# bxh1/VIDO-SLAM

Hardware: AMD Instinct MI355X
Metric: frames/sec end-to-end (flow+depth+track+local-BA) at 640x480; BA iters/sec (higher is better)
Workload: dtype f32

## Files before the change

vido-slam_amd/csrc/detpost.hip:

```cpp
#include "common.hpp"
#include <cfloat>

namespace {
typedef unsigned long long u64;

__device__ void block_sort_desc(u64* keys, int n)
{
    for (int k = 2; k <= n; k <<= 1)
        for (int j = k >> 1; j > 0; j >>= 1) {
            for (int t = threadIdx.x; t < n; t += blockDim.x) {
                const int x = t ^ j;
                if (x > t) {
                    const u64 a = keys[t], b = keys[x];
                    const bool up = (t & k) != 0;
                    if (up ? a > b : a < b) { keys[t] = b; keys[x] = a; }
                }
            }
            __syncthreads();
        }
}

__device__ int block_excl_scan(int v, int* wsum , int* total)
{
    const int lane = threadIdx.x & 63, wave = threadIdx.x >> 6, nw = blockDim.x >> 6;
// ... 182 lines not shown
        const u64 key = mkeys[t];
        int rank = q;
        for (int m = 0; m < Lv; m++) {
            if (m == l) continue;
            const u64* lst = mkeys + (size_t)m * K; int lo = 0, hi = s_cnt[m];
            while (lo < hi) { const int mid = (lo + hi) >> 1; if (lst[mid] > key) lo = mid + 1; else hi = mid; }
            rank += lo;
        }
        if (rank < n_final) {
            const int flat = (int)(0xffffffffu - (unsigned)key);
            for (int c = 0; c < 4; c++) out_boxes[4 * rank + c] = boxes[4 * (size_t)flat + c];
            out_scores[rank] = __uint_as_float((unsigned)(key >> 32));
        }
    }
    if (tid == 0) *n_valid = min(total, n_final);
}

__global__ __launch_bounds__(1024) void k_det_class_sort(const float* __restrict__ prob, const float* __restrict__ deltas, const float* __restrict__ proposals, const float* __restrict__ objectness,
                                                         int N, int nc, float thresh, float wx, float wy, float ww, float wh, float img_w, float img_h,
                                                         float* __restrict__ seg_boxes , int* __restrict__ order , int* __restrict__ seg_n)
{
    __shared__ u64 keys[1024];
    __shared__ int s_n;
    const int j = blockIdx.x + 1, tid = threadIdx.x;
    if (tid == 0) s_n = 0;
    __syncthreads();
    u64 key = 0;
    if (tid < N) {
        float s = prob[(size_t)tid * nc + j];
        if (objectness && objectness[tid] < 0.f) s = 0.f;
        if (s > thresh) { key = ((u64)__float_as_uint(s) << 32) | (u64)(0xffffffffu - (unsigned)tid); atomicAdd(&s_n, 1); }
    }
    keys[tid] = key;
    __syncthreads();
    block_sort_desc(keys, 1024);
    const int n = s_n;
    if (tid < N) {
        float* ob = seg_boxes + ((size_t)(j - 1) * N + tid) * 4; int* oo = order + (size_t)(j - 1) * N + tid;
        if (tid < n) {
            const int i = (int)(0xffffffffu - (unsigned)keys[tid]);
            const float* d = deltas + ((size_t)i * nc + j) * 4;
            decode_clip(proposals + 4 * (size_t)i, d[0], d[1], d[2], d[3], wx, wy, ww, wh, img_w, img_h, ob);
            *oo = i;
        } else { ob[0] = ob[1] = ob[2] = ob[3] = 0.f; *oo = 0; }
    }
    if (tid == 0) seg_n[j - 1] = n;
}

#define DT_STAGE 8192
__global__ __launch_bounds__(1024) void k_det_thresh(const float* __restrict__ prob, const int* __restrict__ order, const int* __restrict__ keep, const int* __restrict__ cnt,
                                                     int N, int nc, int kth, unsigned* __restrict__ thr_out)
{
    __shared__ unsigned hist[256];
    __shared__ unsigned stage[DT_STAGE];
    __shared__ int coff[1025];
    __shared__ unsigned s_prefix, s_kk;
    const int tid = threadIdx.x, lane = tid & 63, wave = tid >> 6, ncls = nc - 1;
    if (tid == 0) { int run = 0; for (int j = 0; j < ncls && j < 1024; j++) { coff[j] = run; run += cnt[j]; } coff[min(ncls, 1024)] = run; }
    __syncthreads();
    const unsigned total = (unsigned)coff[min(ncls, 1024)];
    if (kth <= 0 || total <= (unsigned)kth || ncls > 1024) { if (tid == 0) { thr_out[0] = 0u; thr_out[1] = total; } return; }
    const bool staged = total <= DT_STAGE;
    auto score_bits = [&](int j, int q) { const int i = order[(size_t)j * N + keep[(size_t)j * N + q]]; return __float_as_uint(prob[(size_t)i * nc + j + 1]); };
    if (staged) {
        for (int j = wave; j < ncls; j += 16) { const int c = coff[j + 1] - coff[j]; for (int q = lane; q < c; q += 64) stage[coff[j] + q] = score_bits(j, q); }
        __syncthreads();
    }
    unsigned prefix = 0, mask = 0;
    if (tid == 0) s_kk = (unsigned)kth;
    for (int shift = 24; shift >= 0; shift -= 8) {
        if (tid < 256) hist[tid] = 0;
        __syncthreads();
        if (staged) { for (unsigned t = tid; t < total; t += 1024) { const unsigned u = stage[t]; if ((u & mask) == prefix) atomicAdd(&hist[(u >> shift) & 255u], 1u); } }
        else for (int j = wave; j < ncls; j += 16) { const int c = coff[j + 1] - coff[j]; for (int q = lane; q < c; q += 64) { const unsigned u = score_bits(j, q); if ((u & mask) == prefix) atomicAdd(&hist[(u >> shift) & 255u], 1u); } }
        __syncthreads();
        if (tid == 0) { unsigned kk = s_kk, d; pick_digit_desc(hist, kk, d); s_kk = kk; s_prefix = prefix | (d << shift); }
        __syncthreads();
        prefix = s_prefix; mask |= 0xffu << shift;
    }
    if (tid == 0) { thr_out[0] = prefix; thr_out[1] = total; }
}

__global__ __launch_bounds__(1024) void k_det_emit(const float* __restrict__ prob, const float* __restrict__ seg_boxes, const int* __restrict__ order, const int* __restrict__ keep,
                                                   const int* __restrict__ cnt, int N, int nc, const unsigned* __restrict__ thr, int emit, int* __restrict__ class_counts, int cap,
                                                   float* __restrict__ out_boxes, float* __restrict__ out_scores, long long* __restrict__ out_labels, int* __restrict__ n_det)
{
    __shared__ int flag[1024]; __shared__ int spos[1024]; __shared__ int wsum[17];
    const int j = blockIdx.x, tid = threadIdx.x, ncls = nc - 1;
    const unsigned T = thr[0];
    flag[tid] = 0; spos[tid] = 0;
    __syncthreads();
    const int c = cnt[j];
    for (int q = tid; q < c; q += 1024) {
        const int p = keep[(size_t)j * N + q], i = order[(size_t)j * N + p];
        if (__float_as_uint(prob[(size_t)i * nc + j + 1]) >= T) { flag[i] = 1; spos[i] = p; }
    }
    __syncthreads();
    int total = 0;
    const int rank = block_excl_scan(tid < N ? flag[tid] : 0, wsum, &total);
    if (!emit) { if (tid == 0) class_counts[j] = total; return; }
    int off = 0, all = 0;
    for (int jj = 0; jj < ncls; jj++) { const int t = class_counts[jj]; if (jj < j) off += t; all += t; }
    if (tid < N && flag[tid]) {
        const int slot = off + rank;
        if (slot < cap) {
            const float* b = seg_boxes + ((size_t)j * N + spos[tid]) * 4;
            for (int k = 0; k < 4; k++) out_boxes[4 * slot + k] = b[k];
            out_scores[slot] = prob[(size_t)tid * nc + j + 1]; out_labels[slot] = (long long)(j + 1);
        }
    }
    if (j == 0) {
        for (int s = min(all, cap) + tid; s < cap; s += 1024) { for (int k = 0; k < 4; k++) out_boxes[4 * s + k] = 0.f; out_scores[s] = 0.f; out_labels[s] = 0; }
        if (tid == 0) *n_det = all;
    }
}
}

extern "C" {

int vido_rpn_select(vido_ctx* ctx, int n_levels, const float* const* logits, const float* const* deltas, const int* h, const int* w, const int* stride, const float* cell_anchors,
                    int A, int K, int img_w, int img_h, float* boxes_out, float* scores_out, int32_t* n_out)
{
    if (!ctx) return VIDO_E_INVALID;
    if (n_levels < 1 || n_levels > 8 || A < 1 || A > 4 || K < 1 || K > 1024 || !logits || !deltas || !h || !w || !stride || !cell_anchors || !boxes_out || !scores_out || !n_out)
        return vido_set_error(ctx, VIDO_E_INVALID, "rpn_select: bad arguments (<= 8 levels, <= 4 anchors per cell, K <= 1024)");
    HIP_TRY(ctx, hipSetDevice(ctx->device));
    hipStream_t st = ctx->has_ext_stream ? ctx->ext_stream : ctx->stream;
    RpnLevels L; memset(&L, 0, sizeof L); int maxn = 0; int n_of[8] = {0, 0, 0, 0, 0, 0, 0, 0};
    for (int l = 0; l < n_levels; l++) {
// ... 80 lines not shown
```

vido-slam_amd/csrc/nets.hip:

```cpp
#include "common.hpp"
#include <numeric>

#define CORR_CH 8
__global__ __launch_bounds__(256) void k_correlation(const float* __restrict__ f1, const float* __restrict__ f2, int C, int H, int W, int s,
                                                     int Ho, int Wo, float* __restrict__ out, int nsplit, int cper)
{
    __shared__ float t2[CORR_CH][22][23];
    const int tx = threadIdx.x & 15, ty = threadIdx.x >> 4, b = blockIdx.z / nsplit, split = blockIdx.z - b * nsplit;
    const int c_lo = split * cper, c_hi = min(C, c_lo + cper);
    const int x = blockIdx.x * 16 + tx, y = blockIdx.y * 16 + ty;
    const bool valid = x < Wo && y < Ho;
    float acc[49];
#pragma unroll
    for (int k = 0; k < 49; k++) acc[k] = 0.f;
    const size_t plane = (size_t)H * W;
    for (int c0 = c_lo; c0 < c_hi; c0 += CORR_CH) {
        const int nc = min(CORR_CH, c_hi - c0);
        for (int i = threadIdx.x; i < nc * 22 * 22; i += 256) {
            const int cc = i / (22 * 22), r = (i / 22) % 22, q = i % 22;
            const int yy = (blockIdx.y * 16 + r - 3), xx = (blockIdx.x * 16 + q - 3);
            float v = 0.f;
            if (yy >= 0 && yy < Ho && xx >= 0 && xx < Wo) v = f2[((size_t)b * C + c0 + cc) * plane + (size_t)(yy * s) * W + xx * s];
            t2[cc][r][q] = v;
        }
// ... 178 lines not shown
        const int ph = bin / PW, pw = bin - ph * PW;
        float acc = 0.f;
        if (SR == 2) {
            int o[4][4]; float w[4][4], v[4][4]; bool out[4];
#pragma unroll
            for (int s2 = 0; s2 < 4; s2++) {
                const int iy = s2 >> 1, ix = s2 & 1;
                const float y = sh + ph * bh + (float)(iy + .5f) * bh / (float)gh, x = sw + pw * bw + (float)(ix + .5f) * bw / (float)gw;
                out[s2] = taps(y, x, o[s2][0], o[s2][1], o[s2][2], o[s2][3], w[s2][0], w[s2][1], w[s2][2], w[s2][3]);
            }
#pragma unroll
            for (int s2 = 0; s2 < 4; s2++)
#pragma unroll
                for (int t = 0; t < 4; t++) v[s2][t] = d[(size_t)o[s2][t] * C];
#pragma unroll
            for (int s2 = 0; s2 < 4; s2++) acc += out[s2] ? 0.f : (w[s2][0] * v[s2][0] + w[s2][1] * v[s2][1] + w[s2][2] * v[s2][2] + w[s2][3] * v[s2][3]);
        } else {
            for (int iy = 0; iy < gh; iy++) {
                const float y = sh + ph * bh + (float)(iy + .5f) * bh / (float)gh;
                for (int ix = 0; ix < gw; ix++) {
                    const float x = sw + pw * bw + (float)(ix + .5f) * bw / (float)gw;
                    int o1, o2, o3, o4; float w1, w2, w3, w4;
                    if (taps(y, x, o1, o2, o3, o4, w1, w2, w3, w4)) { acc += 0.f; continue; }
                    const float v1 = d[(size_t)o1 * C], v2 = d[(size_t)o2 * C], v3 = d[(size_t)o3 * C], v4 = d[(size_t)o4 * C];
                    acc += (w1 * v1 + w2 * v2 + w3 * v3 + w4 * v4);
                }
            }
        }
        rl_tile[lane * pitch + bin] = acc / count;
    }
    __syncthreads();
    const int nc = min(64, C - c0), total = nc * nbin;
    float* o = out + ((size_t)i * C + c0) * nbin;
    for (int e = threadIdx.x; e < total; e += 256) { const int cc = e / nbin; o[e] = rl_tile[cc * pitch + (e - cc * nbin)]; }
}
__global__ __launch_bounds__(256) void k_nchw_to_nhwc(const float* __restrict__ src, int C, int HW, float* __restrict__ dst)
{
    __shared__ float t[64][65];
    const int p0 = blockIdx.x * 64, c0 = blockIdx.y * 64, b = blockIdx.z, lane = threadIdx.x & 63, q = threadIdx.x >> 6;
    const float* s = src + (size_t)b * C * HW; float* d = dst + (size_t)b * HW * C;
    for (int k = q; k < 64; k += 4) if (c0 + k < C && p0 + lane < HW) t[k][lane] = s[(size_t)(c0 + k) * HW + p0 + lane];
    __syncthreads();
    for (int k = q; k < 64; k += 4) if (p0 + k < HW && c0 + lane < C) d[(size_t)(p0 + k) * C + c0 + lane] = t[lane][k];
}

__device__ __forceinline__ void tile_of(int t, int nb, int& rb, int& cb)
{
    int r = (int)((2.0f * nb + 1.0f - sqrtf((2.0f * nb + 1.0f) * (2.0f * nb + 1.0f) - 8.0f * (float)t)) * 0.5f);
    r = max(0, min(r, nb - 1));
    while (r > 0 && r * nb - r * (r - 1) / 2 > t) r--;
    while ((r + 1) * nb - (r + 1) * r / 2 <= t) r++;
    rb = r; cb = r + (t - (r * nb - r * (r - 1) / 2));
}
__device__ __forceinline__ void nms_tile(const float* __restrict__ boxes, const int* __restrict__ group, int n, float thresh, unsigned long long* __restrict__ mask, int col_blocks, int rb, int cb, int lane)
{
    const int col = cb * 64 + lane; const bool cv = col < n;
    const float4 b = cv ? *(const float4*)(boxes + 4 * (size_t)col) : make_float4(0.f, 0.f, 0.f, 0.f);
    const float Sb = (b.z - b.x + 1) * (b.w - b.y + 1);
    const int gb = (group && cv) ? group[col] : 0;
    const int rows = min(n - rb * 64, 64);
    unsigned long long mine = 0;
    for (int i = 0; i < rows; i++) {
        const float* a = boxes + 4 * (size_t)(rb * 64 + i);
        const float a0 = a[0], a1 = a[1], a2 = a[2], a3 = a[3];
        const int ga = group ? group[rb * 64 + i] : 0;
        const float left = fmaxf(a0, b.x), right = fminf(a2, b.z), top = fmaxf(a1, b.y), bottom = fminf(a3, b.w);
        const float w = fmaxf(right - left + 1, 0.f), h = fmaxf(bottom - top + 1, 0.f), inter = w * h;
        const float Sa = (a2 - a0 + 1) * (a3 - a1 + 1);
        const bool hit = cv && ga == gb && inter / (Sa + Sb - inter) > thresh;
        unsigned long long word = __ballot(hit);
        if (rb == cb) word &= i >= 63 ? 0ull : ~((2ull << i) - 1ull);
        if (lane == i) mine = word;
    }
    if (lane < rows) mask[(size_t)(rb * 64 + lane) * col_blocks + cb] = mine;
}
__global__ __launch_bounds__(256) void k_nms_mask(const float* __restrict__ boxes, const int* __restrict__ group , int n, float thresh,
                                                 unsigned long long* __restrict__ mask, int col_blocks)
{
    const int t = __builtin_amdgcn_readfirstlane(blockIdx.x * 4 + (threadIdx.x >> 6)), nb = col_blocks;
    if (t >= nb * (nb + 1) / 2) return;
    int rb, cb; tile_of(t, nb, rb, cb);
    nms_tile(boxes, group, n, thresh, mask, col_blocks, rb, cb, threadIdx.x & 63);
}
__global__ __launch_bounds__(64) void k_nms_sweep(const unsigned long long* __restrict__ mask, int n, int col_blocks, int* __restrict__ keep, int* __restrict__ n_keep)
{
    const int lane = threadIdx.x;
    int cnt = 0;
    unsigned long long remv[16];
    const int wpl = (col_blocks + 63) / 64;
    for (int k = 0; k < 16; k++) remv[k] = 0;
    for (int i = 0; i < n; i++) {
        const int nblock = i >> 6, inblock = i & 63;
        const int owner = nblock & 63, slot = nblock >> 6;
        unsigned long long word = 0;
#pragma unroll
        for (int k = 0; k < 16; k++) if (k == slot) word = remv[k];
        word = __shfl(word, owner, 64);
        if (!(word & (1ULL << inblock))) {
            if (lane == 0) keep[cnt] = i;
            cnt++;
            const unsigned long long* p = mask + (size_t)i * col_blocks;
#pragma unroll
            for (int k = 0; k < 16; k++) if (k < wpl) { const int w = k * 64 + lane; if (w >= nblock && w < col_blocks) remv[k] |= p[w]; }
        }
    }
    if (lane == 0) *n_keep = cnt;
}

__global__ __launch_bounds__(64) void k_nms_sweep_seg(const unsigned long long* __restrict__ mask, const int* __restrict__ seg_off, const int* __restrict__ seg_n, int col_blocks,
                                                      int* __restrict__ keep, int* __restrict__ n_keep, int keep_stride)
{
    const int g = blockIdx.x, lane = threadIdx.x;
    const int n = seg_n[g];
    const unsigned long long* M = mask + (size_t)seg_off[g] * col_blocks;
    int* kp = keep + (size_t)g * keep_stride;
    const int cb = (n + 63) >> 6;
    unsigned long long remv[16];
#pragma unroll
    for (int k = 0; k < 16; k++) remv[k] = 0;
    int cnt = 0;
    for (int blk = 0; blk < cb; blk++) {
        const int owner = blk & 63, slot = blk >> 6, rows = min(n - blk * 64, 64);
        unsigned long long word = 0;
#pragma unroll
        for (int k = 0; k < 16; k++) if (k == slot) word = remv[k];
        word = __shfl(word, owner, 64);
        const unsigned long long diag = lane < rows ? M[(size_t)(blk * 64 + lane) * col_blocks + blk] : 0ull;
        const uint32_t dlo = (uint32_t)diag, dhi = (uint32_t)(diag >> 32);
        unsigned long long alive = ~word;
        if (rows < 64) alive &= (1ull << rows) - 1ull;
        unsigned long long keepmask = 0;
        while (alive) {
            const int j = __builtin_ctzll(alive);
            keepmask |= 1ull << j;
            const unsigned long long dj = (unsigned long long)(uint32_t)__builtin_amdgcn_readlane((int)dlo, j) | ((unsigned long long)(uint32_t)__builtin_amdgcn_readlane((int)dhi, j) << 32);
            alive &= ~dj; alive &= ~(1ull << j);
        }
        if ((keepmask >> lane) & 1ull) kp[cnt + __popcll(keepmask & ((1ull << lane) - 1ull))] = blk * 64 + lane;
        cnt += __popcll(keepmask);
        const bool mine = (keepmask >> lane) & 1ull;
        const unsigned long long* prow = M + (size_t)(blk * 64 + lane) * col_blocks;
        for (int w0 = blk + 1; w0 < cb; w0 += 4) {
            unsigned long long v[4];
#pragma unroll
            for (int u = 0; u < 4; u++) v[u] = (mine && w0 + u < cb) ? prow[w0 + u] : 0ull;
#pragma unroll
            for (int u = 0; u < 4; u++) {
                uint32_t lo = (uint32_t)v[u], hi = (uint32_t)(v[u] >> 32);
#pragma unroll
                for (int o = 32; o >= 1; o >>= 1) { lo |= (uint32_t)__shfl_xor((int)lo, o, 64); hi |= (uint32_t)__shfl_xor((int)hi, o, 64); }
                const int w = w0 + u;
                if (w < cb && lane == (w & 63)) {
                    const unsigned long long r = (unsigned long long)lo | ((unsigned long long)hi << 32);
#pragma unroll
                    for (int k = 0; k < 16; k++) if (k == (w >> 6)) remv[k] |= r;
                }
            }
        }
    }
    for (int i = cnt + lane; i < keep_stride; i += 64) kp[i] = -1;
    if (lane == 0) n_keep[g] = cnt;
}
__global__ __launch_bounds__(256) void k_nms_mask_seg(const float* __restrict__ boxes, const int* __restrict__ group, const int* __restrict__ seg_off, const int* __restrict__ seg_n,
                                                     float thresh, unsigned long long* __restrict__ mask, int col_blocks)
{
    const int g = blockIdx.y, n = seg_n[g], off = seg_off[g];
    const int nb = (n + 63) >> 6, t = __builtin_amdgcn_readfirstlane(blockIdx.x * 4 + (threadIdx.x >> 6));
    if (t >= nb * (nb + 1) / 2) return;
    int rb, cb; tile_of(t, nb, rb, cb);
    nms_tile(boxes + 4 * (size_t)off, group ? group + off : nullptr, n, thresh, mask + (size_t)off * col_blocks, col_blocks, rb, cb, threadIdx.x & 63);
}

struct PasteDet { int x0, y0, w, h, label; float rw, rh; };
__global__ __launch_bounds__(256) void k_paste_prepare(const float* __restrict__ boxes, const int64_t* __restrict__ labels, int n, int M, int padding, PasteDet* __restrict__ det)
{
    const int i = blockIdx.x * blockDim.x + threadIdx.x;
    if (i >= n) return;
    const float scale = (float)((double)(M + 2 * padding) / (double)M);
    const float* b = boxes + 4 * (size_t)i;
    const float wh = (b[2] - b[0]) * 0.5f * scale, hh = (b[3] - b[1]) * 0.5f * scale;
    const float xc = (b[2] + b[0]) * 0.5f, yc = (b[3] + b[1]) * 0.5f;
    const int x0 = (int)(xc - wh), y0 = (int)(yc - hh), x1 = (int)(xc + wh), y1 = (int)(yc + hh);
    PasteDet d; d.x0 = x0; d.y0 = y0; d.w = max(x1 - x0 + 1, 1); d.h = max(y1 - y0 + 1, 1); d.label = (int)labels[i];
    const int Mp = M + 2 * padding;
    d.rw = (float)Mp / (float)d.w; d.rh = (float)Mp / (float)d.h;
    det[i] = d;
}
__global__ __launch_bounds__(256) void k_paste_label(const float* __restrict__ masks , const PasteDet* __restrict__ det, int n, int M, int padding, float thresh,
                                                     int H, int W, uint8_t* __restrict__ out)
{
    __shared__ PasteDet sd[128];
    const int x = blockIdx.x * 32 + (threadIdx.x & 31), y = blockIdx.y * 8 + (threadIdx.x >> 5);
    const int Mp = M + 2 * padding;
    unsigned acc = 0;
    for (int d0 = 0; d0 < n; d0 += 128) {
        __syncthreads();
        if ((int)threadIdx.x < min(128, n - d0)) sd[threadIdx.x] = det[d0 + threadIdx.x];
        __syncthreads();
        if (x < W && y < H) {
            for (int k = 0; k < min(128, n - d0); k++) {
                const PasteDet d = sd[k];
                const int u = x - d.x0, v = y - d.y0;
                if (u < 0 || v < 0 || u >= d.w || v >= d.h) continue;
                float sy = d.rh * ((float)v + 0.5f) - 0.5f; if (sy < 0.f) sy = 0.f;
                float sx = d.rw * ((float)u + 0.5f) - 0.5f; if (sx < 0.f) sx = 0.f;
                const int iy = (int)sy, ix = (int)sx; const int iyp = iy < Mp - 1 ? 1 : 0, ixp = ix < Mp - 1 ? 1 : 0;
                const float ly = sy - (float)iy, lx = sx - (float)ix, hy = 1.f - ly, hx = 1.f - lx;
                const float* m = masks + (size_t)(d0 + k) * M * M;
                auto at = [&](int yy, int xx) -> float { yy -= padding; xx -= padding; return (yy < 0 || xx < 0 || yy >= M || xx >= M) ? 0.f : m[yy * M + xx]; };
                const float val = hy * (hx * at(iy, ix) + lx * at(iy, ix + ixp)) + ly * (hx * at(iy + iyp, ix) + lx * at(iy + iyp, ix + ixp));
                if (val > thresh) acc += (unsigned)d.label;
            }
        }
    }
    if (x < W && y < H) out[(size_t)y * W + x] = (uint8_t)acc;
}

__global__ void k_zero_i32(int32_t* __restrict__ p, int n)
{
    const int i = blockIdx.x * blockDim.x + threadIdx.x;
    if (i < n) p[i] = 0;
}
__global__ __launch_bounds__(256) void k_paste_instance(const float* __restrict__ masks , const PasteDet* __restrict__ det, int n, int M, int padding, float thresh,
// ... 173 lines not shown
    if (w >= W || h >= H) return;
    const size_t hw = (size_t)H * W, o = (size_t)h * W + w;
    const float* dp = dist + (size_t)b * ND * hw + o;
    float e[ND]; float m = -INFINITY;
#pragma unroll
    for (int c = 0; c < ND; c++) { const float v = dp[(size_t)c * hw]; e[c] = -(v * v); m = fmaxf(m, e[c]); }
    const float* fxp = flow + (size_t)b * 2 * hw; const float* fyp = fxp + hw;
    float s = 0.f, ax = 0.f, ay = 0.f;
#pragma unroll
    for (int c = 0; c < ND; c++) {
        const float p = expf(e[c] - m);
        s += p;
        const int yy = h + c / K - PAD, xx = w + c % K - PAD;
        const bool in = yy >= 0 && yy < H && xx >= 0 && xx < W;
        const size_t q = in ? (size_t)yy * W + xx : 0;
        const float ux = in ? fxp[q] : 0.f, uy = in ? fyp[q] : 0.f;
        ax += wx[c] * (p * ux); ay += wy[c] * (p * uy);
    }
    const float div = 1.0f / s;
    out[(size_t)b * 2 * hw + o] = (ax + bx[0]) * div;
    out[(size_t)b * 2 * hw + hw + o] = (ay + by[0]) * div;
}

__global__ __launch_bounds__(256) void k_deconv4s2_dw(const float* __restrict__ in, const float* __restrict__ wgt , int C, int H, int W, float slope, float* __restrict__ out)
{
    const int OW = 2 * W, OH = 2 * H;
    const int ox = blockIdx.x * 64 + (threadIdx.x & 63), oy = blockIdx.y * 4 + (threadIdx.x >> 6), bc = blockIdx.z, c = bc % C;
    if (ox >= OW || oy >= OH) return;
    const float* ip = in + (size_t)bc * H * W; const float* wp = wgt + 16 * c;
    const int ky0 = (oy + 1) & 1, kx0 = (ox + 1) & 1, iy0 = (oy + 1 - ky0) >> 1, ix0 = (ox + 1 - kx0) >> 1;
    float acc = 0.f;
#pragma unroll
    for (int a = 0; a < 2; a++) {
        const int iy = iy0 - a, ky = ky0 + 2 * a;
#pragma unroll
        for (int b = 0; b < 2; b++) {
            const int ix = ix0 - b, kx = kx0 + 2 * b;
            if (iy >= 0 && iy < H && ix >= 0 && ix < W) { float v = ip[(size_t)iy * W + ix]; v = v > 0.f ? v : v * slope; acc += v * wp[ky * 4 + kx]; }
        }
    }
    out[((size_t)bc * OH + oy) * OW + ox] = acc;
}

static int roi_lds_limit(vido_ctx* ctx, size_t lds)
{
    static size_t have = 48 * 1024;
    if (lds <= have) return VIDO_OK;
    HIP_TRY(ctx, hipFuncSetAttribute((const void*)k_roi_align_nhwc<2>, hipFuncAttributeMaxDynamicSharedMemorySize, (int)lds));
    HIP_TRY(ctx, hipFuncSetAttribute((const void*)k_roi_align_nhwc<0>, hipFuncAttributeMaxDynamicSharedMemorySize, (int)lds));
    have = lds;
    return VIDO_OK;
}

extern "C" {

int vido_correlation(vido_ctx* ctx, const float* first, const float* second, int B, int C, int H, int W, int stride, float* out, int on_device)
{
    if (!ctx) return VIDO_E_INVALID;
    if (!first || !second || !out || B < 1 || C < 1 || H < 1 || W < 1 || (stride != 1 && stride != 2)) return vido_set_error(ctx, VIDO_E_INVALID, "correlation: bad arguments");
    HIP_TRY(ctx, hipSetDevice(ctx->device));
    hipStream_t st = (on_device && ctx->has_ext_stream) ? ctx->ext_stream : ctx->stream;
    const int Ho = (H + stride - 1) / stride, Wo = (W + stride - 1) / stride;
    const size_t nin = (size_t)B * C * H * W * 4, nout = (size_t)B * 49 * Ho * Wo * 4;
    const float *d1 = first, *d2 = second; float* dout = out;
    const int tiles = ((Wo + 15) / 16) * ((Ho + 15) / 16) * B, nchunk = (C + CORR_CH - 1) / CORR_CH;
    int nsplit = std::max(1, std::min(nchunk, 512 / std::max(tiles, 1)));
    const int cper = ((nchunk + nsplit - 1) / nsplit) * CORR_CH; nsplit = (C + cper - 1) / cper;
    const size_t nel = (size_t)B * 49 * Ho * Wo, io_bytes = on_device ? 0 : 2 * al256(nin) + al256(nout), pbytes = nsplit > 1 ? al256(nel * 4 * nsplit) : 0;
    NetState* S = nullptr;
    if (io_bytes + pbytes) { int rc = net_scratch(ctx, io_bytes + pbytes, &S); if (rc) return rc; }
    if (!on_device) {
        memcpy(S->h, first, nin); memcpy(S->h + al256(nin), second, nin);
        HIP_TRY(ctx, hipMemcpyAsync(S->d, S->h, 2 * al256(nin), hipMemcpyHostToDevice, st));
        d1 = (float*)S->d; d2 = (float*)(S->d + al256(nin)); dout = (float*)(S->d + 2 * al256(nin));
    }
    if (nsplit == 1) hipLaunchKernelGGL(k_correlation, dim3((Wo + 15) / 16, (Ho + 15) / 16, B), dim3(256), 0, st, d1, d2, C, H, W, stride, Ho, Wo, dout, 1, C);
    else {
        float* part = (float*)(S->d + io_bytes);
        hipLaunchKernelGGL(k_correlation, dim3((Wo + 15) / 16, (Ho + 15) / 16, B * nsplit), dim3(256), 0, st, d1, d2, C, H, W, stride, Ho, Wo, part, nsplit, cper);
        hipLaunchKernelGGL(k_correlation_reduce, dim3((unsigned)((nel + 255) / 256)), dim3(256), 0, st, (const float*)part, nsplit, nel, 0.f, C, dout);
    }
    HIP_TRY(ctx, hipGetLastError());
    if (!on_device) {
        HIP_TRY(ctx, hipStreamSynchronize(st));
        HIP_TRY(ctx, hipMemcpyAsync(S->h, dout, nout, hipMemcpyDeviceToHost, st)); HIP_TRY(ctx, hipStreamSynchronize(st));
        memcpy(out, S->h, nout);
    }
    return VIDO_OK;
}

int vido_det_order(vido_ctx* ctx, const float* scores, const long long* labels, const int* n_det, float confidence, int cap, long long* order, long long* labels_out, long long* n_live)
{
    return vido_det_order_n(ctx, scores, labels, n_det, confidence, cap, order, labels_out, n_live, nullptr);
}
int vido_det_order_n(vido_ctx* ctx, const float* scores, const long long* labels, const int* n_det, float confidence, int cap, long long* order, long long* labels_out, long long* n_live,
                     int32_t* n_live32)
{
    if (!ctx) return VIDO_E_INVALID;
    if (!scores || !labels || !n_det || !order || !labels_out || !n_live || cap < 1 || cap > 1024) return vido_set_error(ctx, VIDO_E_INVALID, "det_order: bad arguments (cap 1 .. 1024)");
    HIP_TRY(ctx, hipSetDevice(ctx->device));
    hipStream_t st = ctx->has_ext_stream ? ctx->ext_stream : ctx->stream;
    hipLaunchKernelGGL(k_det_order, dim3(1), dim3(1024), 0, st, scores, labels, n_det, confidence, cap, order, labels_out, n_live, n_live32);
    HIP_TRY(ctx, hipGetLastError());
    return VIDO_OK;
}

// ... 202 lines not shown
    NetState* S = nullptr;
    int rc = net_scratch(ctx, al256(nb) + al256(nm) + al256(nk) + al256(ng), &S); if (rc) return rc;
    const int* dgroups = groups;
    const float* dboxes = boxes_xyxy; unsigned long long* dmask = (unsigned long long*)(S->d + al256(nb));
    int* dkeep = keep_out; int* dn = n_keep;
    std::vector<int> order;
    if (!on_device) {
        order.resize(n); std::iota(order.begin(), order.end(), 0);
        std::stable_sort(order.begin(), order.end(), [&](int a, int b) { return scores[a] > scores[b]; });
        float* hb = (float*)S->h;
        for (int i = 0; i < n; i++) memcpy(hb + 4 * (size_t)i, boxes_xyxy + 4 * (size_t)order[i], 16);
        HIP_TRY(ctx, hipMemcpyAsync(S->d, S->h, nb, hipMemcpyHostToDevice, st));
        dboxes = (float*)S->d; dkeep = (int*)(S->d + al256(nb) + al256(nm)); dn = dkeep + n;
        if (groups) {
            int* hg = (int*)(S->h + al256(nb)); for (int i = 0; i < n; i++) hg[i] = groups[order[i]];
            int* dg = (int*)(S->d + al256(nb) + al256(nm) + al256(nk));
            HIP_TRY(ctx, hipMemcpyAsync(dg, hg, ng, hipMemcpyHostToDevice, st)); dgroups = dg;
        }
    }
    hipLaunchKernelGGL(k_nms_mask, dim3((cb * (cb + 1) / 2 + 3) / 4), dim3(256), 0, st, dboxes, dgroups, n, thresh, dmask, cb);
    hipLaunchKernelGGL(k_nms_sweep, dim3(1), dim3(64), 0, st, dmask, n, cb, dkeep, dn);
    HIP_TRY(ctx, hipGetLastError());
    if (!on_device) {
        HIP_TRY(ctx, hipStreamSynchronize(st));
        HIP_TRY(ctx, hipMemcpyAsync(S->h, dkeep, nk, hipMemcpyDeviceToHost, st)); HIP_TRY(ctx, hipStreamSynchronize(st));
        const int* hk = (const int*)S->h; const int m = hk[n];
        for (int i = 0; i < m; i++) keep_out[i] = order[hk[i]];
        std::sort(keep_out, keep_out + m);
        *n_keep = m;
    }
    return VIDO_OK;
}

int vido_nms(vido_ctx* ctx, const float* boxes_xyxy, const float* scores, int n, float thresh, int32_t* keep_out, int32_t* n_keep, int on_device)
{
    return nms_impl(ctx, boxes_xyxy, scores, nullptr, n, thresh, keep_out, n_keep, on_device);
}
int vido_nms_grouped(vido_ctx* ctx, const float* boxes_xyxy, const float* scores, const int32_t* groups, int n, float thresh,
                     int32_t* keep_out, int32_t* n_keep, int on_device)
{
    if (n > 0 && !groups) return ctx ? vido_set_error(ctx, VIDO_E_INVALID, "nms_grouped: null groups") : VIDO_E_INVALID;
    return nms_impl(ctx, boxes_xyxy, scores, groups, n, thresh, keep_out, n_keep, on_device);
}

int vido_nms_segments(vido_ctx* ctx, const float* boxes_xyxy, const int32_t* groups, const int32_t* seg_off, const int32_t* seg_n, int n_seg, int max_n, int total,
                      float thresh, int32_t* keep_out, int32_t* n_keep)
{
    if (!ctx) return VIDO_E_INVALID;
    if (!boxes_xyxy || !seg_off || !seg_n || !keep_out || !n_keep || n_seg < 1 || max_n < 1 || total < 1) return vido_set_error(ctx, VIDO_E_INVALID, "nms_segments: bad arguments");
    if (max_n > 65536) return vido_set_error(ctx, VIDO_E_CAPACITY, "nms_segments: %d boxes per segment > 65536", max_n);
    HIP_TRY(ctx, hipSetDevice(ctx->device));
    hipStream_t st = ctx->has_ext_stream ? ctx->ext_stream : ctx->stream;
    const int cb = (max_n + 63) / 64;
    NetState* S = nullptr;
    int rc = net_scratch(ctx, al256((size_t)total * cb * 8), &S); if (rc) return rc;
    unsigned long long* dmask = (unsigned long long*)S->d;
    hipLaunchKernelGGL(k_nms_mask_seg, dim3((cb * (cb + 1) / 2 + 3) / 4, n_seg), dim3(256), 0, st, boxes_xyxy, groups, seg_off, seg_n, thresh, dmask, cb);
    hipLaunchKernelGGL(k_nms_sweep_seg, dim3(n_seg), dim3(64), 0, st, dmask, seg_off, seg_n, cb, keep_out, n_keep, max_n);
    HIP_TRY(ctx, hipGetLastError());
    return VIDO_OK;
}

int vido_roi_align_fpn(vido_ctx* ctx, const float* const feat[4], const int H[4], const int W[4], const float scale[4], int C, const float* boxes, const int32_t* level,
                       int n, int pooled_h, int pooled_w, int sampling_ratio, float* out)
{
    if (!ctx) return VIDO_E_INVALID;
    if (!feat || !H || !W || !scale || C < 1 || n < 0 || pooled_h < 1 || pooled_w < 1 || (n && (!boxes || !level || !out))) return vido_set_error(ctx, VIDO_E_INVALID, "roi_align_fpn: bad arguments");
    if (n == 0) return VIDO_OK;
    HIP_TRY(ctx, hipSetDevice(ctx->device));
    hipStream_t st = ctx->has_ext_stream ? ctx->ext_stream : ctx->stream;
    size_t off[5] = {0, 0, 0, 0, 0};
    for (int l = 0; l < 4; l++) off[l + 1] = off[l] + al256((size_t)C * H[l] * W[l] * 4);
    NetState* S = nullptr;
    { int rc = net_scratch(ctx, off[4], &S); if (rc) return rc; }
    const float* nh[4];
    for (int l = 0; l < 4; l++) {
        hipLaunchKernelGGL(k_nchw_to_nhwc, dim3((H[l] * W[l] + 63) / 64, (C + 63) / 64, 1), dim3(256), 0, st, feat[l], C, H[l] * W[l], (float*)(S->d + off[l]));
        nh[l] = (const float*)(S->d + off[l]);
    }
    return vido_roi_align_fpn_nhwc(ctx, nh, H, W, scale, C, boxes, level, n, pooled_h, pooled_w, sampling_ratio, out);
}

int vido_roi_align_fpn_nhwc(vido_ctx* ctx, const float* const feat[4], const int H[4], const int W[4], const float scale[4], int C, const float* boxes, const int32_t* level,
                            int n, int pooled_h, int pooled_w, int sampling_ratio, float* out)
{
    return vido_roi_align_fpn_nhwc_n(ctx, feat, H, W, scale, C, boxes, level, n, pooled_h, pooled_w, sampling_ratio, out, nullptr);
}
int vido_roi_align_fpn_nhwc_n(vido_ctx* ctx, const float* const feat[4], const int H[4], const int W[4], const float scale[4], int C, const float* boxes, const int32_t* level,
                              int n, int pooled_h, int pooled_w, int sampling_ratio, float* out, const int32_t* n_live)
{
    if (!ctx) return VIDO_E_INVALID;
    if (!feat || !H || !W || !scale || C < 1 || n < 0 || pooled_h < 1 || pooled_w < 1 || (n && (!boxes || !level || !out))) return vido_set_error(ctx, VIDO_E_INVALID, "roi_align_fpn_nhwc: bad arguments");
    if (n == 0) return VIDO_OK;
    HIP_TRY(ctx, hipSetDevice(ctx->device));
    hipStream_t st = ctx->has_ext_stream ? ctx->ext_stream : ctx->stream;
    RoiLevels L;
    for (int l = 0; l < 4; l++) { L.feat[l] = feat[l]; L.H[l] = H[l]; L.W[l] = W[l]; L.scale[l] = scale[l]; }
    const size_t lds = (size_t)64 * ((pooled_h * pooled_w) | 1) * sizeof(float);
    if (lds > 150 * 1024) return vido_set_error(ctx, VIDO_E_CAPACITY, "roi_align_fpn: pooled size %d x %d too large", pooled_h, pooled_w);
    { int rc = roi_lds_limit(ctx, lds); if (rc) return rc; }
    if (sampling_ratio == 2) hipLaunchKernelGGL(k_roi_align_nhwc<2>, dim3(n, (C + 63) / 64), dim3(256), lds, st, L, C, boxes, 4, level, pooled_h, pooled_w, sampling_ratio, out, n_live);
    else hipLaunchKernelGGL(k_roi_align_nhwc<0>, dim3(n, (C + 63) / 64), dim3(256), lds, st, L, C, boxes, 4, level, pooled_h, pooled_w, sampling_ratio, out, n_live);
    HIP_TRY(ctx, hipGetLastError());
    return VIDO_OK;
}

int vido_mask_label_image(vido_ctx* ctx, const float* masks, const float* boxes, const int64_t* labels, int n, int M, int padding, float thresh, int H, int W, uint8_t* out)
{
    if (!ctx) return VIDO_E_INVALID;
    if (!out || H < 1 || W < 1 || n < 0 || M < 1 || padding < 0 || (n && (!masks || !boxes || !labels))) return vido_set_error(ctx, VIDO_E_INVALID, "mask_label_image: bad arguments");
    HIP_TRY(ctx, hipSetDevice(ctx->device));
// ... 59 lines not shown
```

Before: 131.7.

## Parallelize detection top-k threshold and segmented NMS sweep via LDS and wave ops

The top-k score threshold kernel now builds class offsets with a block-wide scan instead of a serial thread-0 loop. For up to 1024 candidates it bitonic-sorts in shared memory rather than doing radix passes, and digit selection uses a wave-level shuffle scan instead of a single thread. Segmented NMS splits each 64x64 IoU tile across four waves, broadcasts row boxes with readlane, and emits transposed diagonal masks. A new LDS-resident sweep kernel uses ballot-based fixed-point iteration to resolve each 64-box block in parallel, replacing the serial per-box sweep. This adds shared-memory pressure and more complex code paths, gated by segment size, the absence of groups, and an environment switch.

```diff
diff --git a/vido-slam_amd/csrc/detpost.hip b/vido-slam_amd/csrc/detpost.hip
--- a/vido-slam_amd/csrc/detpost.hip
+++ b/vido-slam_amd/csrc/detpost.hip
@@ -258,16 +258,30 @@
                                                      int N, int nc, int kth, unsigned* __restrict__ thr_out)
 {
     __shared__ unsigned hist[256];
-    __shared__ unsigned stage[DT_STAGE];
+    __shared__ __attribute__((aligned(16))) unsigned stage[DT_STAGE];
     __shared__ int coff[1025];
+    __shared__ int wsum[17];
     __shared__ unsigned s_prefix, s_kk;
-    const int tid = threadIdx.x, lane = tid & 63, wave = tid >> 6, ncls = nc - 1;
-    if (tid == 0) { int run = 0; for (int j = 0; j < ncls && j < 1024; j++) { coff[j] = run; run += cnt[j]; } coff[min(ncls, 1024)] = run; }
-    __syncthreads();
-    const unsigned total = (unsigned)coff[min(ncls, 1024)];
+    const int tid = threadIdx.x, lane = tid & 63, wave = tid >> 6, ncls = nc - 1, nj = min(ncls, 1024);
+    int tot;
+    const int before = block_excl_scan(tid < nj ? cnt[tid] : 0, wsum, &tot);
+    if (tid < nj) coff[tid] = before;
+    if (tid == 0) coff[nj] = tot;
+    __syncthreads();
+    const unsigned total = (unsigned)tot;
     if (kth <= 0 || total <= (unsigned)kth || ncls > 1024) { if (tid == 0) { thr_out[0] = 0u; thr_out[1] = total; } return; }
     const bool staged = total <= DT_STAGE;
     auto score_bits = [&](int j, int q) { const int i = order[(size_t)j * N + keep[(size_t)j * N + q]]; return __float_as_uint(prob[(size_t)i * nc + j + 1]); };
+    if (total <= 1024) {
+        u64* keys = (u64*)stage;
+        keys[tid] = 0;
+        __syncthreads();
+        for (int j = wave; j < ncls; j += 16) { const int c = coff[j + 1] - coff[j]; for (int q = lane; q < c; q += 64) keys[coff[j] + q] = (u64)score_bits(j, q) << 32; }
+        __syncthreads();
+        block_sort_desc(keys, 1024);
+        if (tid == 0) { thr_out[0] = (unsigned)(keys[kth - 1] >> 32); thr_out[1] = total; }
+        return;
+    }
     if (staged) {
         for (int j = wave; j < ncls; j += 16) { const int c = coff[j + 1] - coff[j]; for (int q = lane; q < c; q += 64) stage[coff[j] + q] = score_bits(j, q); }
         __syncthreads();
@@ -280,7 +294,22 @@
         if (staged) { for (unsigned t = tid; t < total; t += 1024) { const unsigned u = stage[t]; if ((u & mask) == prefix) atomicAdd(&hist[(u >> shift) & 255u], 1u); } }
         else for (int j = wave; j < ncls; j += 16) { const int c = coff[j + 1] - coff[j]; for (int q = lane; q < c; q += 64) { const unsigned u = score_bits(j, q); if ((u & mask) == prefix) atomicAdd(&hist[(u >> shift) & 255u], 1u); } }
         __syncthreads();
-        if (tid == 0) { unsigned kk = s_kk, d; pick_digit_desc(hist, kk, d); s_kk = kk; s_prefix = prefix | (d << shift); }
+        if (wave == 0) {
+            const unsigned kk = s_kk;
+            const unsigned h0 = hist[4 * lane], h1 = hist[4 * lane + 1], h2 = hist[4 * lane + 2], h3 = hist[4 * lane + 3];
+            unsigned incl = h0 + h1 + h2 + h3;
+#pragma unroll
+            for (int o = 1; o < 64; o <<= 1) { const unsigned t = (unsigned)__shfl_down((int)incl, o, 64); if (lane + o < 64) incl += t; }
+            unsigned above = incl - (h0 + h1 + h2 + h3);
+            const unsigned hs[4] = {h3, h2, h1, h0};
+            bool found = false;
+#pragma unroll
+            for (int b = 0; b < 4; b++) {
+                if (!found && kk > above && kk <= above + hs[b]) { found = true; s_kk = kk - above; s_prefix = prefix | ((unsigned)(4 * lane + 3 - b) << shift); }
+                above += hs[b];
+            }
+            if (!__ballot(found) && lane == 0) { s_kk = kk - incl; s_prefix = prefix; }
+        }
         __syncthreads();
         prefix = s_prefix; mask |= 0xffu << shift;
     }
diff --git a/vido-slam_amd/csrc/nets.hip b/vido-slam_amd/csrc/nets.hip
--- a/vido-slam_amd/csrc/nets.hip
+++ b/vido-slam_amd/csrc/nets.hip
@@ -254,27 +254,36 @@
     while ((r + 1) * nb - (r + 1) * r / 2 <= t) r++;
     rb = r; cb = r + (t - (r * nb - r * (r - 1) / 2));
 }
-__device__ __forceinline__ void nms_tile(const float* __restrict__ boxes, const int* __restrict__ group, int n, float thresh, unsigned long long* __restrict__ mask, int col_blocks, int rb, int cb, int lane)
+__device__ __forceinline__ unsigned long long nms_tile_word(const float* __restrict__ boxes, const int* __restrict__ group, int n, float thresh, int rb, int cb, int lane, unsigned long long& colT,
+                                                            int i0 = 0, int i1 = 64)
 {
     const int col = cb * 64 + lane; const bool cv = col < n;
     const float4 b = cv ? *(const float4*)(boxes + 4 * (size_t)col) : make_float4(0.f, 0.f, 0.f, 0.f);
     const float Sb = (b.z - b.x + 1) * (b.w - b.y + 1);
     const int gb = (group && cv) ? group[col] : 0;
     const int rows = min(n - rb * 64, 64);
+    const float4 rbx = lane < rows ? *(const float4*)(boxes + 4 * (size_t)(rb * 64 + lane)) : make_float4(0.f, 0.f, 0.f, 0.f);
     unsigned long long mine = 0;
-    for (int i = 0; i < rows; i++) {
-        const float* a = boxes + 4 * (size_t)(rb * 64 + i);
-        const float a0 = a[0], a1 = a[1], a2 = a[2], a3 = a[3];
+    colT = 0;
+    for (int i = i0; i < min(rows, i1); i++) {
+        const float a0 = __int_as_float(__builtin_amdgcn_readlane(__float_as_int(rbx.x), i)), a1 = __int_as_float(__builtin_amdgcn_readlane(__float_as_int(rbx.y), i)),
+                    a2 = __int_as_float(__builtin_amdgcn_readlane(__float_as_int(rbx.z), i)), a3 = __int_as_float(__builtin_amdgcn_readlane(__float_as_int(rbx.w), i));
         const int ga = group ? group[rb * 64 + i] : 0;
         const float left = fmaxf(a0, b.x), right = fminf(a2, b.z), top = fmaxf(a1, b.y), bottom = fminf(a3, b.w);
         const float w = fmaxf(right - left + 1, 0.f), h = fmaxf(bottom - top + 1, 0.f), inter = w * h;
         const float Sa = (a2 - a0 + 1) * (a3 - a1 + 1);
         const bool hit = cv && ga == gb && inter / (Sa + Sb - inter) > thresh;
         unsigned long long word = __ballot(hit);
-        if (rb == cb) word &= i >= 63 ? 0ull : ~((2ull << i) - 1ull);
+        if (rb == cb) { word &= i >= 63 ? 0ull : ~((2ull << i) - 1ull); colT |= (hit && lane > i) ? (1ull << i) : 0ull; }
         if (lane == i) mine = word;
     }
-    if (lane < rows) mask[(size_t)(rb * 64 + lane) * col_blocks + cb] = mine;
+    return mine;
+}
+__device__ __forceinline__ void nms_tile(const float* __restrict__ boxes, const int* __restrict__ group, int n, float thresh, unsigned long long* __restrict__ mask, int col_blocks, int rb, int cb, int lane)
+{
+    unsigned long long colT;
+    const unsigned long long mine = nms_tile_word(boxes, group, n, thresh, rb, cb, lane, colT);
+    if (lane < min(n - rb * 64, 64)) mask[(size_t)(rb * 64 + lane) * col_blocks + cb] = mine;
 }
 __global__ __launch_bounds__(256) void k_nms_mask(const float* __restrict__ boxes, const int* __restrict__ group , int n, float thresh,
                                                  unsigned long long* __restrict__ mask, int col_blocks)
@@ -364,13 +373,81 @@
     if (lane == 0) n_keep[g] = cnt;
 }
 __global__ __launch_bounds__(256) void k_nms_mask_seg(const float* __restrict__ boxes, const int* __restrict__ group, const int* __restrict__ seg_off, const int* __restrict__ seg_n,
-                                                     float thresh, unsigned long long* __restrict__ mask, int col_blocks)
-{
+                                                     float thresh, unsigned long long* __restrict__ mask, int col_blocks, unsigned long long* __restrict__ diagT )
+{
+    __shared__ unsigned long long sT[4][64];
     const int g = blockIdx.y, n = seg_n[g], off = seg_off[g];
-    const int nb = (n + 63) >> 6, t = __builtin_amdgcn_readfirstlane(blockIdx.x * 4 + (threadIdx.x >> 6));
+    const int nb = (n + 63) >> 6, t = blockIdx.x, q = __builtin_amdgcn_readfirstlane(threadIdx.x >> 6), lane = threadIdx.x & 63;
     if (t >= nb * (nb + 1) / 2) return;
     int rb, cb; tile_of(t, nb, rb, cb);
-    nms_tile(boxes + 4 * (size_t)off, group ? group + off : nullptr, n, thresh, mask + (size_t)off * col_blocks, col_blocks, rb, cb, threadIdx.x & 63);
+    unsigned long long colT;
+    const unsigned long long mine = nms_tile_word(boxes + 4 * (size_t)off, group ? group + off : nullptr, n, thresh, rb, cb, lane, colT, q * 16, q * 16 + 16);
+    const int rows = min(n - rb * 64, 64);
+    if (lane < rows && (lane >> 4) == q) mask[((size_t)off + rb * 64 + lane) * col_blocks + cb] = mine;
+    if (diagT && rb == cb) {
+        sT[q][lane] = colT;
+        __syncthreads();
+        if (q == 0 && lane < rows) diagT[(size_t)off + rb * 64 + lane] = sT[0][lane] | sT[1][lane] | sT[2][lane] | sT[3][lane];
+    }
+}
+
+#define NMS_TP 66
+#define NMS_LDS_MAX_N 1024
+#define NMS_LDS_BYTES(cb) ((size_t)((cb) * ((cb) + 1) / 2) * NMS_TP * 8)
+__device__ __forceinline__ void nms_sweep_lds(const unsigned long long* __restrict__ tri, int n, int* __restrict__ kp, int keep_stride, int* __restrict__ n_keep, int lane)
+{
+    const int nb = (n + 63) >> 6, wcol = lane >> 2, q = lane & 3;
+    unsigned long long remv = 0;
+    int cnt = 0;
+    for (int blk = 0, tb = 0; blk < nb; tb += nb - blk, blk++) {
+        const int rows = min(n - blk * 64, 64);
+        const unsigned long long word = __shfl(remv, 4 * blk, 64);
+        const unsigned long long colT = lane < rows ? tri[(size_t)tb * NMS_TP + lane] : 0ull;
+        unsigned long long alive = ~word;
+        if (rows < 64) alive &= (1ull << rows) - 1ull;
+        unsigned long long keepmask = alive;
+        for (;;) {
+            const unsigned long long next = alive & ~__ballot((colT & keepmask) != 0ull);
+            if (next == keepmask) break;
+            keepmask = next;
+        }
+        if ((keepmask >> lane) & 1ull) kp[cnt + __popcll(keepmask & ((1ull << lane) - 1ull))] = blk * 64 + lane;
+        cnt += __popcll(keepmask);
+        unsigned long long acc = 0;
+        if (wcol > blk && wcol < nb) {
+            const unsigned long long* t = tri + (size_t)(tb + wcol - blk) * NMS_TP + q * 16;
+#pragma unroll
+            for (int i = 0; i < 16; i++) { const unsigned long long v = t[i]; acc |= ((keepmask >> (q * 16 + i)) & 1ull) ? v : 0ull; }
+        }
+        uint32_t lo = (uint32_t)acc, hi = (uint32_t)(acc >> 32);
+#pragma unroll
+        for (int o = 2; o >= 1; o >>= 1) { lo |= (uint32_t)__shfl_xor((int)lo, o, 64); hi |= (uint32_t)__shfl_xor((int)hi, o, 64); }
+        remv |= (unsigned long long)lo | ((unsigned long long)hi << 32);
+    }
+    for (int i = cnt + lane; i < keep_stride; i += 64) kp[i] = -1;
+    if (lane == 0) *n_keep = cnt;
+}
+__global__ __launch_bounds__(1024) void k_nms_sweep_seg_lds(const unsigned long long* __restrict__ mask, const unsigned long long* __restrict__ diagT, const int* __restrict__ seg_off,
+                                                            const int* __restrict__ seg_n, int col_blocks, int* __restrict__ keep, int* __restrict__ n_keep, int keep_stride)
+{
+    extern __shared__ __attribute__((aligned(16))) unsigned long long nms_tri[];
+    const int g = blockIdx.x, lane = threadIdx.x & 63;
+    const int n = min(seg_n[g], keep_stride);
+    int* kp = keep + (size_t)g * keep_stride;
+    if (n <= 0) {
+        for (int i = threadIdx.x; i < keep_stride; i += 1024) kp[i] = -1;
+        if (threadIdx.x == 0) n_keep[g] = 0;
+        return;
+    }
+    const unsigned long long* M = mask + (size_t)seg_off[g] * col_blocks;
+    const unsigned long long* T = diagT + seg_off[g];
+    const int nb = (n + 63) >> 6;
+    for (int e = threadIdx.x; e < n * col_blocks; e += 1024) {
+        const int row = e / col_blocks, w = e - row * col_blocks, rb = row >> 6;
+        if (w >= rb && w < nb) nms_tri[(size_t)(rb * nb - rb * (rb - 1) / 2 + (w - rb)) * NMS_TP + (row & 63)] = w == rb ? T[row] : M[e];
+    }
+    __syncthreads();
+    if (threadIdx.x < 64) nms_sweep_lds(nms_tri, n, kp, keep_stride, n_keep + g, lane);
 }
 
 struct PasteDet { int x0, y0, w, h, label; float rw, rh; };
@@ -650,6 +727,15 @@
     return VIDO_OK;
 }
 
+static int nms_lds_limit(vido_ctx* ctx)
+{
+    static bool done = false;
+    if (done) return VIDO_OK;
+    HIP_TRY(ctx, hipFuncSetAttribute((const void*)k_nms_sweep_seg_lds, hipFuncAttributeMaxDynamicSharedMemorySize, (int)NMS_LDS_BYTES(NMS_LDS_MAX_N / 64)));
+    done = true;
+    return VIDO_OK;
+}
+
 extern "C" {
 
 int vido_correlation(vido_ctx* ctx, const float* first, const float* second, int B, int C, int H, int W, int stride, float* out, int on_device)
@@ -958,11 +1044,16 @@
     HIP_TRY(ctx, hipSetDevice(ctx->device));
     hipStream_t st = ctx->has_ext_stream ? ctx->ext_stream : ctx->stream;
     const int cb = (max_n + 63) / 64;
+    const char* sw = getenv("VIDO_NMS_LDS");
+    const bool lds = max_n <= NMS_LDS_MAX_N && !groups && !(sw && !strcmp(sw, "0"));
+    if (lds) { int rc = nms_lds_limit(ctx); if (rc) return rc; }
     NetState* S = nullptr;
-    int rc = net_scratch(ctx, al256((size_t)total * cb * 8), &S); if (rc) return rc;
-    unsigned long long* dmask = (unsigned long long*)S->d;
-    hipLaunchKernelGGL(k_nms_mask_seg, dim3((cb * (cb + 1) / 2 + 3) / 4, n_seg), dim3(256), 0, st, boxes_xyxy, groups, seg_off, seg_n, thresh, dmask, cb);
-    hipLaunchKernelGGL(k_nms_sweep_seg, dim3(n_seg), dim3(64), 0, st, dmask, seg_off, seg_n, cb, keep_out, n_keep, max_n);
+    const size_t nm = al256((size_t)total * cb * 8);
+    int rc = net_scratch(ctx, nm + al256((size_t)total * 8), &S); if (rc) return rc;
+    unsigned long long* dmask = (unsigned long long*)S->d; unsigned long long* dT = lds ? (unsigned long long*)(S->d + nm) : nullptr;
+    hipLaunchKernelGGL(k_nms_mask_seg, dim3(cb * (cb + 1) / 2, n_seg), dim3(256), 0, st, boxes_xyxy, groups, seg_off, seg_n, thresh, dmask, cb, dT);
+    if (lds) hipLaunchKernelGGL(k_nms_sweep_seg_lds, dim3(n_seg), dim3(1024), NMS_LDS_BYTES(cb), st, dmask, dT, seg_off, seg_n, cb, keep_out, n_keep, max_n);
+    else hipLaunchKernelGGL(k_nms_sweep_seg, dim3(n_seg), dim3(64), 0, st, dmask, seg_off, seg_n, cb, keep_out, n_keep, max_n);
     HIP_TRY(ctx, hipGetLastError());
     return VIDO_OK;
 }
```

Measured after the change: 131.6. No clear change (-0.1%).
